# bifurcationkit/BifurcationKit.jl

Measured on NVIDIA H100. Metric: continuation steps/sec (SH2d PALC), higher is better.
Workload: dtype f64

## Files before the change

bifurcationkit.jl_b200/csrc/bk_fft_fast.cuh:

```cuda
#pragma once
#include "bk_common.cuh"
#include "bk_async.cuh"

namespace bkf {

template <int LOGN_, int LOGE_>
struct Cfg {
  static constexpr int LOGN = LOGN_, LOGE = LOGE_;
  static constexpr int N = 1 << LOGN, E = 1 << LOGE, T = N / E;
  static constexpr int F = LOGN / LOGE, RB = LOGN % LOGE;
  static constexpr int NP = F + (RB ? 1 : 0);
  static constexpr int PP = (T >= 32) ? 2 : 64 / T;
  static constexpr int THREADS = T * PP;
  static constexpr int PB = LOGE == 5 ? (LOGN >= 10 ? 5 : 4) : LOGE == 4 ? 4 : LOGE == 3 ? ((LOGN == 9 || LOGN == 10) ? 3 : 0) : 0;
  __host__ __device__ static constexpr int pad(int i) { return i + (i >> 2) + (PB ? (i >> PB) : 0); }
  static constexpr int TPSM = LOGE == 5 ? 256 : LOGE == 4 ? 512 : LOGE == 3 ? 768 : 1024;
  static constexpr int MINB = TPSM / THREADS > 0 ? TPSM / THREADS : 1;
  static constexpr int MINB_P = MINB > 1 ? MINB - 1 : 1;
  static constexpr int NB = LOGE == 2 ? (LOGN <= 6 ? 0 : LOGN <= 8 ? 4 : LOGN <= 10 ? 6 : 8)
                          : LOGE == 3 ? (LOGN <= 6 ? 0 : LOGN <= 9 ? 3 : 6)
                          : LOGE == 4 ? (LOGN <= 8 ? 0 : 4)
                                      : (LOGN <= 10 ? 0 : 5);
  __host__ __device__ static constexpr int padn(int k) { return k + (k >> 2) + (NB ? (k >> NB) : 0); }
  static constexpr int SLOTS_POS = pad(N - 1) + 1, SLOTS_NAT = padn(N - 1) + 1;
  static constexpr int SLOTS = SLOTS_POS > SLOTS_NAT ? SLOTS_POS : SLOTS_NAT;
  static constexpr size_t SMEM_DATA = sizeof(double2) * (size_t)SLOTS * PP;
  __host__ __device__ static constexpr int logr(int p) { return p < F ? LOGE : RB; }
  __host__ __device__ static constexpr int logNp(int p) { return LOGN - LOGE * p; }
  __host__ __device__ static constexpr int logMp(int p) { return logNp(p) - logr(p); }
  __host__ __device__ static constexpr int tw_off(int p) {
    int o = 0;
    for (int q = 0; q < p; ++q) o += ((1 << logr(q)) - 1) << logMp(q);
    return o;
  }
  static constexpr int TW_TOTAL = tw_off(NP);
  static constexpr size_t SMEM = SMEM_DATA + sizeof(double2) * ((size_t)TW_TOTAL + N);
  static constexpr size_t SMEM_FUSED = SMEM + sizeof(double2) * (size_t)N;
  static_assert(LOGN >= LOGE + 1 && LOGN <= 11, "line length out of range");
  static_assert(THREADS <= 1024, "CTA too large");
};

template <class C>
__host__ __device__ inline int k_of_pos(int p) {
  int k = 0, sh = 0;
  for (int q = 0; q < C::NP; ++q) {
    const int d = (p >> C::logMp(q)) & ((1 << C::logr(q)) - 1);
    k |= d << sh;
    sh += C::logr(q);
  }
  return k;
}
template <class C>
__host__ __device__ inline int pos_of_k(int k) {
  int p = 0, sh = 0;
  for (int q = 0; q < C::NP; ++q) {
    const int d = (k >> sh) & ((1 << C::logr(q)) - 1);
    p |= d << C::logMp(q);
    sh += C::logr(q);
  }
  return p;
}
__host__ __device__ constexpr int brev_c(int j, int bits) {
  int r = 0;
  for (int b = 0; b < bits; ++b) r |= ((j >> b) & 1) << (bits - 1 - b);
  return r;
}

#ifdef __CUDACC__
__device__ __forceinline__ double2 cadd(double2 a, double2 b) { return make_double2(a.x + b.x, a.y + b.y); }
__device__ __forceinline__ double2 csub(double2 a, double2 b) { return make_double2(a.x - b.x, a.y - b.y); }
__device__ __forceinline__ double2 cmul(double2 a, double2 b) {
  return make_double2(fma(a.x, b.x, -(a.y * b.y)), fma(a.x, b.y, a.y * b.x));
}
__device__ __forceinline__ double2 cmulc(double2 a, double2 b) {
  return make_double2(fma(a.x, b.x, a.y * b.y), fma(a.y, b.x, -(a.x * b.y)));
}

#define BKF_C1 0.98078528040323043
#define BKF_S1 0.19509032201612825
#define BKF_C2 0.92387953251128674
#define BKF_S2 0.38268343236508978
#define BKF_C3 0.83146961230254524
#define BKF_S3 0.55557023301960218
#define BKF_C4 0.70710678118654752
template <bool INV>
__device__ __forceinline__ double2 mul_w32(double2 t, int j) {
  double c, s;
  switch (j) {
    case 0: return t;
    case 8: return INV ? make_double2(-t.y, t.x) : make_double2(t.y, -t.x);
    case 4: {
      const double a = BKF_C4 * t.x, b = BKF_C4 * t.y;
      return INV ? make_double2(a - b, a + b) : make_double2(a + b, b - a);
    }
    case 12: {
      const double a = BKF_C4 * t.x, b = BKF_C4 * t.y;
      return INV ? make_double2(-a - b, a - b) : make_double2(b - a, -a - b);
    }
    case 1: c = BKF_C1; s = BKF_S1; break;
    case 2: c = BKF_C2; s = BKF_S2; break;
    case 3: c = BKF_C3; s = BKF_S3; break;
    case 5: c = BKF_S3; s = BKF_C3; break;
    case 6: c = BKF_S2; s = BKF_C2; break;
    case 7: c = BKF_S1; s = BKF_C1; break;
    case 9: c = -BKF_S1; s = BKF_C1; break;
    case 10: c = -BKF_S2; s = BKF_C2; break;
    case 11: c = -BKF_S3; s = BKF_C3; break;
    case 13: c = -BKF_C3; s = BKF_S3; break;
    case 14: c = -BKF_C2; s = BKF_S2; break;
    default: c = -BKF_C1; s = BKF_S1; break;
  }
  return INV ? make_double2(fma(t.x, c, -(t.y * s)), fma(t.y, c, t.x * s)) : make_double2(fma(t.x, c, t.y * s), fma(t.y, c, -(t.x * s)));
}

template <int R, int S0, int ESZ>
__device__ __forceinline__ void bfly_fwd(double2 (&a)[ESZ]) {
  if constexpr (R >= 2) {
    constexpr int H = R / 2;
#pragma unroll
    for (int i = 0; i < H; ++i) {
      const double2 u = a[S0 + i], v = a[S0 + i + H];
      a[S0 + i] = cadd(u, v);
      a[S0 + i + H] = mul_w32<false>(csub(u, v), i * (32 / R));
    }
    bfly_fwd<H, S0, ESZ>(a);
    bfly_fwd<H, S0 + H, ESZ>(a);
  }
}
template <int R, int S0, int ESZ>
__device__ __forceinline__ void bfly_inv(double2 (&a)[ESZ]) {
  if constexpr (R >= 2) {
    constexpr int H = R / 2;
    bfly_inv<H, S0, ESZ>(a);
    bfly_inv<H, S0 + H, ESZ>(a);
#pragma unroll
    for (int i = 0; i < H; ++i) {
      const double2 u = a[S0 + i], t = mul_w32<true>(a[S0 + i + H], i * (32 / R));
      a[S0 + i] = cadd(u, t);
      a[S0 + i + H] = csub(u, t);
    }
  }
}

struct Tables {
  const double2* tw;
  const double2* om;
  const double2* lam2;
};
template <class C, bool FUSED>
__device__ __forceinline__ Tables stage_tables(const Tables& g, double2* sm, unsigned long long* bar) {
  Tables t;
  double2* stw = sm + (size_t)C::SLOTS * C::PP;
  double2* som = stw + C::TW_TOTAL;
  double2* slam = som + C::N;
  if (threadIdx.x == 0) {
    mbar_init(bar, 1);
    fence_mbar_init();
    constexpr unsigned twb = 16u * C::TW_TOTAL, nb = 16u * C::N;
    mbar_arrive_expect_tx(bar, twb + nb + (FUSED ? nb : 0u));
    if (twb) bulk_g2s(stw, g.tw, twb, bar);
    bulk_g2s(som, g.om, nb, bar);
    if (FUSED) bulk_g2s(slam, g.lam2, nb, bar);
  }
  t.tw = stw;
  t.om = som;
  t.lam2 = slam;
  return t;
}

struct Geom {
  long long es;
  long long os;
  int nb;
  int nouter;
};

struct Symbol {
  const double* lam_b;
  const double* lam_o;
  double shift;
  double scale;
  const double* tail_src;
  double* tail_dst;
  int tail_n;
  int neg;
};

template <class C>
__device__ __forceinline__ int slot(int pos, int pr) { return C::pad(pos) * C::PP + pr; }

template <class C, int P>
__device__ __forceinline__ void pass_geom(int tau, int u, int& base, int& b) {
  constexpr int LM = C::logMp(P), LN = C::logNp(P);
  const int beta = tau + C::T * u;
  const int blk = beta >> LM;
  b = beta & ((1 << LM) - 1);
  base = (blk << LN) + b;
}

template <int R, int U, int NB, int ESZ>
__device__ __forceinline__ void bfly_all_fwd(double2 (&a)[ESZ]) {
  if constexpr (U < NB) {
    bfly_fwd<R, U * R, ESZ>(a);
    bfly_all_fwd<R, U + 1, NB, ESZ>(a);
  }
}
template <int R, int U, int NB, int ESZ>
__device__ __forceinline__ void bfly_all_inv(double2 (&a)[ESZ]) {
  if constexpr (U < NB) {
    bfly_inv<R, U * R, ESZ>(a);
    bfly_all_inv<R, U + 1, NB, ESZ>(a);
  }
}

template <class C, int P>
__device__ __forceinline__ void fwd_passes(double2 (&a)[C::E], double2* sm, const Tables& tb, int tau, int pr) {
  constexpr int LR = C::logr(P), R = 1 << LR, NB = C::E / R, LM = C::logMp(P);
  if constexpr (P > 0) {
#pragma unroll
    for (int u = 0; u < NB; ++u) {
      int base, b;
      pass_geom<C, P>(tau, u, base, b);
#pragma unroll
      for (int i = 0; i < R; ++i) a[u * R + i] = sm[slot<C>(base + (i << LM), pr)];
    }
  }
  bfly_all_fwd<R, 0, NB, C::E>(a);
  if constexpr (P < C::NP - 1) {
    const double2* tw = tb.tw + C::tw_off(P);
#pragma unroll
    for (int u = 0; u < NB; ++u) {
      int base, b;
      pass_geom<C, P>(tau, u, base, b);
#pragma unroll
      for (int j = 0; j < R; ++j) {
        const int q = brev_c(j, LR);
        double2 v = a[u * R + j];
        if (q > 0) v = cmul(v, tw[((q - 1) << LM) + b]);
        sm[slot<C>(base + (q << LM), pr)] = v;
      }
    }
    __syncthreads();
    fwd_passes<C, P + 1>(a, sm, tb, tau, pr);
  }
}

template <class C, int P>
__device__ __forceinline__ void inv_passes(double2 (&a)[C::E], double2* sm, const Tables& tb, int tau, int pr) {
  constexpr int LR = C::logr(P), R = 1 << LR, NB = C::E / R, LM = C::logMp(P);
  if constexpr (P < C::NP - 1) {
    const double2* tw = tb.tw + C::tw_off(P);
#pragma unroll
    for (int u = 0; u < NB; ++u) {
      int base, b;
      pass_geom<C, P>(tau, u, base, b);
#pragma unroll
      for (int j = 0; j < R; ++j) {
        const int q = brev_c(j, LR);
        double2 v = sm[slot<C>(base + (q << LM), pr)];
        if (q > 0) v = cmulc(v, tw[((q - 1) << LM) + b]);
        a[u * R + j] = v;
      }
    }
  }
  bfly_all_inv<R, 0, NB, C::E>(a);
  if constexpr (P > 0) {
#pragma unroll
    for (int u = 0; u < NB; ++u) {
      int base, b;
      pass_geom<C, P>(tau, u, base, b);
#pragma unroll
      for (int i = 0; i < R; ++i) sm[slot<C>(base + (i << LM), pr)] = a[u * R + i];
    }
    __syncthreads();
    inv_passes<C, P - 1>(a, sm, tb, tau, pr);
  }
}

template <class C>
__device__ __forceinline__ int reg_pos(int tau, int reg) {
  constexpr int LR = C::logr(C::NP - 1), R = 1 << LR;
  const int u = reg >> LR, j = reg & (R - 1);
  return ((tau + C::T * u) << LR) + brev_c(j, LR);
}
template <class C>
__device__ __forceinline__ void park(const double2 (&a)[C::E], double2* sm, int tau, int pr) {
#pragma unroll
  for (int reg = 0; reg < C::E; ++reg) sm[slot<C>(reg_pos<C>(tau, reg), pr)] = a[reg];
}
template <class C>
__device__ __forceinline__ double2 partner(const double2* sm, int pos, int pr, int& k) {
  k = k_of_pos<C>(pos);
  const int nk = (C::N - k) & (C::N - 1);
  return sm[slot<C>(pos_of_k<C>(nk), pr)];
}
template <class C>
__device__ __forceinline__ int row_of(int i, int tau) {
  const int m = i * C::T + tau;
  return (i < C::E / 2) ? 2 * m : 2 * C::N - 1 - 2 * m;
}

template <class C>
__device__ __forceinline__ void strided_load(double2 (&a)[C::E], const double* __restrict__ base, long long es, int tau, bool v0,
                                             bool v1) {
  if (v1) {
#pragma unroll
    for (int i = 0; i < C::E; ++i) a[i] = __ldg(reinterpret_cast<const double2*>(base + (long long)row_of<C>(i, tau) * es));
  } else {
#pragma unroll
    for (int i = 0; i < C::E; ++i) a[i] = make_double2(v0 ? __ldg(base + (long long)row_of<C>(i, tau) * es) : 0.0, 0.0);
  }
}
template <class C>
__device__ __forceinline__ void strided_store(const double2 (&a)[C::E], double* __restrict__ base, long long es, int tau, bool v0,
                                              bool v1) {
  if (v1) {
#pragma unroll
    for (int i = 0; i < C::E; ++i) *reinterpret_cast<double2*>(base + (long long)row_of<C>(i, tau) * es) = a[i];
  } else if (v0) {
#pragma unroll
    for (int i = 0; i < C::E; ++i) base[(long long)row_of<C>(i, tau) * es] = a[i].x;
  }
}

#define BKF_BOUNDS(C, PERIODIC) __launch_bounds__(C::THREADS, (PERIODIC) ? C::MINB_P : C::MINB)

__device__ __forceinline__ double rcp_nr(double x) {
  double r;
  asm("rcp.approx.ftz.f64 %0, %1;" : "=d"(r) : "d"(x));
  double e = fma(-x, r, 1.0);
  r = fma(r, e, r);
  e = fma(-x, r, 1.0);
  return fma(r, e, r);
}
__device__ __forceinline__ double per_symbol(const Symbol& sy, double lam) {
  const double t = 1.0 + lam, l1 = t * t;
  return sy.neg ? -sy.scale * l1 : sy.scale * rcp_nr(l1 + sy.shift);
}

template <class C, int MODE>
static __global__ void BKF_BOUNDS(C, MODE == 3) k_strided(const double* __restrict__ in, double* __restrict__ out, Geom g, Tables tbg, Symbol sy) {
  extern __shared__ __align__(128) double2 sm_fast[];
  __shared__ __align__(8) unsigned long long tbar;
  double2* sm = sm_fast;
  const Tables tb = stage_tables<C, MODE == 2 || MODE == 3>(tbg, sm, &tbar);
  const int tid = threadIdx.x, pr = tid % C::PP, tau = tid / C::PP;
  __syncthreads();
  bk_pdl_sync();
  const int col = (blockIdx.x * C::PP + pr) * 2, o = blockIdx.y;
  const bool v0 = col < g.nb, v1 = col + 1 < g.nb;
  const long long off = (long long)o * g.os + col;
  if ((MODE == 2 || MODE == 3) && sy.tail_n > 0 && blockIdx.x == 0 && blockIdx.y == 0 && tid < sy.tail_n)
    sy.tail_dst[tid] = sy.tail_src[tid];
  double2 a[C::E];
  if (MODE == 3) {
#pragma unroll
    for (int i = 0; i < C::E; ++i) {
      const double* p = in + off + (long long)(i * C::T + tau) * g.es;
      a[i] = v1 ? __ldg(reinterpret_cast<const double2*>(p)) : make_double2(v0 ? __ldg(p) : 0.0, 0.0);
    }
    mbar_wait(&tbar, 0);
    fwd_passes<C, 0>(a, sm, tb, tau, pr);
    const bool nyq = blockIdx.x == 0 && pr == 0;
    if (blockIdx.x == 0) {
      park<C>(a, sm, tau, pr);
      __syncthreads();
      if (nyq) {
        const double l0 = __ldg(sy.lam_b), ln = __ldg(sy.lam_b + (g.nb >> 1));
#pragma unroll
        for (int reg = 0; reg < C::E; ++reg) {
          int k;
          const double2 z = a[reg], zp = partner<C>(sm, reg_pos<C>(tau, reg), pr, k);
          const double ly = tb.lam2[reg * C::T + tau].x;
          const double s0 = per_symbol(sy, l0 + ly), sn = per_symbol(sy, ln + ly);
          const double hp = 0.5 * (s0 + sn), hm = 0.5 * (s0 - sn);
          a[reg] = make_double2(fma(hp, z.x, hm * zp.x), fma(hp, z.y, -(hm * zp.y)));
        }
      }
      __syncthreads();
    }
    if (!nyq) {
      const double lq = v0 ? __ldg(sy.lam_b + (col >> 1)) : 0.0;
#pragma unroll
      for (int reg = 0; reg < C::E; ++reg) {
        const double s = per_symbol(sy, lq + tb.lam2[reg * C::T + tau].x);
        a[reg] = make_double2(s * a[reg].x, s * a[reg].y);
      }
    }
    inv_passes<C, C::NP - 1>(a, sm, tb, tau, pr);
#pragma unroll
    for (int i = 0; i < C::E; ++i) {
      double* p = out + off + (long long)(i * C::T + tau) * g.es;
      if (v1) *reinterpret_cast<double2*>(p) = a[i];
      else if (v0) *p = a[i].x;
    }
    return;
  }
  if (MODE != 1) {
    strided_load<C>(a, in + off, g.es, tau, v0, v1);
    mbar_wait(&tbar, 0);
    fwd_passes<C, 0>(a, sm, tb, tau, pr);
    park<C>(a, sm, tau, pr);
    __syncthreads();
  }
  if (MODE == 0) {
#pragma unroll
    for (int reg = 0; reg < C::E; ++reg) {
      int k;
      const double2 z = a[reg], zp = partner<C>(sm, reg_pos<C>(tau, reg), pr, k);
      const double2 w = tb.om[reg * C::T + tau];
      const double sx = z.x + zp.x, sy_ = z.y - zp.y;
      const double dx = z.x - zp.x, dy = z.y + zp.y;
      const double c1 = fma(w.x, sx, -(w.y * sy_)), c2 = fma(w.x, dy, w.y * dx);
      double* p = out + off + (long long)k * g.es;
      if (v1) *reinterpret_cast<double2*>(p) = make_double2(c1, c2);
      else if (v0) *p = c1;
    }
    return;
  }
  if (MODE == 1) {
#pragma unroll
    for (int reg = 0; reg < C::E; ++reg) {
      const int k = k_of_pos<C>(reg_pos<C>(tau, reg));
      const double* p = in + off + (long long)k * g.es;
      a[reg] = v1 ? __ldg(reinterpret_cast<const double2*>(p)) : make_double2(v0 ? __ldg(p) : 0.0, 0.0);
    }
    mbar_wait(&tbar, 0);
    park<C>(a, sm, tau, pr);
    __syncthreads();
#pragma unroll
    for (int reg = 0; reg < C::E; ++reg) {
      int k;
      double2 dn = partner<C>(sm, reg_pos<C>(tau, reg), pr, k);
      if (k == 0) dn = make_double2(0.0, 0.0);
      const double2 w = tb.om[reg * C::T + tau];
      a[reg] = cmulc(make_double2(a[reg].x + dn.y, a[reg].y - dn.x), w);
    }
    __syncthreads();
  }
  if (MODE == 2) {
    const double lo = sy.lam_o ? __ldg(sy.lam_o + o) : 0.0;
    const double cA = 1.0 + lo + (v0 ? __ldg(sy.lam_b + col) : 0.0), cB = 1.0 + lo + (v1 ? __ldg(sy.lam_b + col + 1) : 0.0);
#pragma unroll
    for (int reg = 0; reg < C::E; ++reg) {
      int k;
      const double2 z = a[reg], zp = partner<C>(sm, reg_pos<C>(tau, reg), pr, k);
      const double2 w = tb.om[reg * C::T + tau];
      const double2 l2 = tb.lam2[reg * C::T + tau];
      const double2 A1 = cmul(make_double2(z.x + zp.x, z.y - zp.y), w);
      const double2 A2 = cmul(make_double2(z.y + zp.y, zp.x - z.x), w);
      double t = cA + l2.x;
      const double s1k = fma(t, t, sy.shift);
      t = cA + l2.y;
      const double s1n = fma(t, t, sy.shift);
      t = cB + l2.x;
      const double s2k = fma(t, t, sy.shift);
      t = cB + l2.y;
      const double s2n = fma(t, t, sy.shift);
      const double r1 = sy.scale * __drcp_rn(s1k * s1n), r2 = sy.scale * __drcp_rn(s2k * s2n);
      const double h1x = A1.x * (r1 * s1n), h1y = A1.y * (r1 * s1k);
      const double h2x = A2.x * (r2 * s2n), h2y = A2.y * (r2 * s2k);
      a[reg] = cmulc(make_double2(h1x - h2y, h1y + h2x), w);
    }
    __syncthreads();
  }
  inv_passes<C, C::NP - 1>(a, sm, tb, tau, pr);
  strided_store<C>(a, out + off, g.es, tau, v0, v1);
}

template <class C>
__device__ __forceinline__ int nslot(int k, int pr) { return C::padn(k) * C::PP + pr; }

__device__ __forceinline__ double pw_c(const PerPw& pw, double u) { return fma(u, fma(-3.0, u, 2.0 * pw.nu), pw.l); }
__device__ __forceinline__ double pw_d(const PerPw& pw, double u) { return fma(pw.a1, pw.spc + pw_c(pw, u), pw.a0); }
__device__ __forceinline__ double pw_out(const PerPw& pw, double y, const double* v, const double* u, int m, double s) {
  switch (pw.epi) {
    case PW_RESID: {
      const double x = __ldg(v + m);
      return fma(x, fma(x, pw.nu - x, pw.l), y);
    }
    case PW_JVP: return fma(fma(pw.a1, pw_c(pw, __ldg(u + m)), pw.a0), s * __ldg(v + m), y);
    case PW_FLEFT: return fma(-pw.a1 * s, __ldg(v + m), y);
    case PW_FRIGHT: return fma(pw_d(pw, __ldg(u + m)), y, -pw.a1 * s * __ldg(v + m));
    default: return y;
  }
}

template <class C, int MODE>
static __global__ void BKF_BOUNDS(C, MODE == 2) k_contig(const double* __restrict__ in, double* __restrict__ out, Geom g, Tables tbg, PerPw pw) {
  extern __shared__ __align__(128) double2 sm_fast[];
  __shared__ __align__(8) unsigned long long tbar;
  double2* sm = sm_fast;
  const Tables tb = stage_tables<C, false>(tbg, sm, &tbar);
  const int tid = threadIdx.x, pr = tid % C::PP, tau = tid / C::PP;
  __syncthreads();
  bk_pdl_sync();
  const long long lineA = ((long long)blockIdx.x * C::PP + pr) * 2, lineB = lineA + 1;
  const bool vA = lineA < g.nb, vB = lineB < g.nb;
  const double* inA = in + lineA * g.os;
  const double* inB = in + lineB * g.os;
  double* outA = out + lineA * g.os;
  double* outB = out + lineB * g.os;
  double2 a[C::E];
  if (MODE == 2) {
    const double s = pw.sp ? __ldg(pw.sp) : 1.0;
#pragma unroll
    for (int i = 0; i < C::E; ++i) {
      const int m = i * C::T + tau;
      double xa = vA ? __ldg(inA + m) : 0.0, xb = vB ? __ldg(inB + m) : 0.0;
      if (pw.pro == PW_D) {
        xa *= vA ? pw_d(pw, __ldg(pw.u + lineA * g.os + m)) : 0.0;
        xb *= vB ? pw_d(pw, __ldg(pw.u + lineB * g.os + m)) : 0.0;
      }
      a[i] = make_double2(s * xa, s * xb);
    }
    mbar_wait(&tbar, 0);
    fwd_passes<C, 0>(a, sm, tb, tau, pr);
    park<C>(a, sm, tau, pr);
    __syncthreads();
    double2 b[C::E];
#pragma unroll
    for (int reg = 0; reg < C::E; ++reg) {
      int k;
      const double2 z = a[reg], zp = partner<C>(sm, reg_pos<C>(tau, reg), pr, k);
      a[reg] = make_double2(0.5 * (z.x + zp.x), 0.5 * (z.y + zp.y));
      b[reg] = make_double2(0.5 * (z.y - zp.y), 0.5 * (zp.x - z.x));
    }
    __syncthreads();
#pragma unroll
    for (int reg = 0; reg < C::E; ++reg) {
      const int k = k_of_pos<C>(reg_pos<C>(tau, reg));
      if (k == 0) sm[nslot<C>(0, pr)] = a[reg];
      else if (k == C::N / 2) sm[nslot<C>(1, pr)] = a[reg];
      else if (k < C::N / 2) {
        sm[nslot<C>(2 * k, pr)] = a[reg];
        sm[nslot<C>(2 * k + 1, pr)] = b[reg];
      }
    }
    __syncthreads();
#pragma unroll
    for (int i = 0; i < C::E; ++i) {
      const int p = i * C::T + tau;
      const double2 d = sm[nslot<C>(p, pr)];
      if (vA) outA[p] = d.x;
      if (vB) outB[p] = d.y;
    }
    return;
  }
  if (MODE == 3) {
#pragma unroll
    for (int i = 0; i < C::E; ++i) {
      const int p = i * C::T + tau;
      sm[nslot<C>(p, pr)] = make_double2(vA ? __ldg(inA + p) : 0.0, vB ? __ldg(inB + p) : 0.0);
    }
    mbar_wait(&tbar, 0);
    __syncthreads();
#pragma unroll
    for (int reg = 0; reg < C::E; ++reg) {
      const int k = k_of_pos<C>(reg_pos<C>(tau, reg)), kk = k <= C::N / 2 ? k : C::N - k;
      double2 xa, xb;
      if (kk == 0 || kk == C::N / 2) {
        const double2 d = sm[nslot<C>(kk ? 1 : 0, pr)];
        xa = make_double2(d.x, 0.0);
        xb = make_double2(d.y, 0.0);
      } else {
        const double2 re = sm[nslot<C>(2 * kk, pr)], im = sm[nslot<C>(2 * kk + 1, pr)];
        xa = make_double2(re.x, k == kk ? im.x : -im.x);
        xb = make_double2(re.y, k == kk ? im.y : -im.y);
      }
      a[reg] = make_double2(xa.x - xb.y, xa.y + xb.x);
    }
    __syncthreads();
    inv_passes<C, C::NP - 1>(a, sm, tb, tau, pr);
    const double s = pw.sp ? __ldg(pw.sp) : 1.0;
    const double* vrA = pw.v + lineA * g.os;
    const double* vrB = pw.v + lineB * g.os;
    const double* urA = pw.u ? pw.u + lineA * g.os : nullptr;
    const double* urB = pw.u ? pw.u + lineB * g.os : nullptr;
#pragma unroll
    for (int i = 0; i < C::E; ++i) {
      const int m = i * C::T + tau;
      if (vA) outA[m] = pw_out(pw, a[i].x, vrA, urA, m, s);
      if (vB) outB[m] = pw_out(pw, a[i].y, vrB, urB, m, s);
    }
    return;
  }
  if (MODE == 0) {
#pragma unroll
    for (int i = 0; i < C::E; ++i) {
      const int e = row_of<C>(i, tau);
      a[i] = make_double2(vA ? __ldg(inA + e) : 0.0, vB ? __ldg(inB + e) : 0.0);
    }
    mbar_wait(&tbar, 0);
    fwd_passes<C, 0>(a, sm, tb, tau, pr);
    park<C>(a, sm, tau, pr);
    __syncthreads();
#pragma unroll
    for (int reg = 0; reg < C::E; ++reg) {
      int k;
      const double2 z = a[reg], zp = partner<C>(sm, reg_pos<C>(tau, reg), pr, k);
      const double2 w = tb.om[reg * C::T + tau];
      const double sx = z.x + zp.x, sy_ = z.y - zp.y, dx = z.x - zp.x, dy = z.y + zp.y;
      a[reg] = make_double2(fma(w.x, sx, -(w.y * sy_)), fma(w.x, dy, w.y * dx));
    }
    __syncthreads();
#pragma unroll
    for (int reg = 0; reg < C::E; ++reg) sm[nslot<C>(k_of_pos<C>(reg_pos<C>(tau, reg)), pr)] = a[reg];
    __syncthreads();
#pragma unroll
    for (int i = 0; i < C::E; ++i) {
      const int k = i * C::T + tau;
      const double2 d = sm[nslot<C>(k, pr)];
      if (vA) outA[k] = d.x;
      if (vB) outB[k] = d.y;
    }
  } else {
#pragma unroll
    for (int i = 0; i < C::E; ++i) {
      const int k = i * C::T + tau;
      sm[nslot<C>(k, pr)] = make_double2(vA ? __ldg(inA + k) : 0.0, vB ? __ldg(inB + k) : 0.0);
    }
    mbar_wait(&tbar, 0);
    __syncthreads();
#pragma unroll
    for (int reg = 0; reg < C::E; ++reg) {
      const int k = k_of_pos<C>(reg_pos<C>(tau, reg)), nk = (C::N - k) & (C::N - 1);
      const double2 w = tb.om[reg * C::T + tau];
      const double2 d = sm[nslot<C>(k, pr)];
      double2 dn = sm[nslot<C>(nk, pr)];
      if (k == 0) dn = make_double2(0.0, 0.0);
      a[reg] = cmulc(make_double2(d.x + dn.y, d.y - dn.x), w);
    }
    __syncthreads();
    inv_passes<C, C::NP - 1>(a, sm, tb, tau, pr);
#pragma unroll
    for (int i = 0; i < C::E; ++i) {
      const int e = row_of<C>(i, tau);
      if (vA) outA[e] = a[i].x;
      if (vB) outB[e] = a[i].y;
    }
  }
}
#endif

template <class C>
static inline void build_tables(std::vector<double>& tw, std::vector<double>& om, std::vector<double>& lam2, const double* lam) {
  const long double PI = 3.14159265358979323846264338327950288L;
  tw.assign(2 * (size_t)C::TW_TOTAL, 0.0);
  for (int p = 0; p < C::NP - 1; ++p) {
    const int r = 1 << C::logr(p), M = 1 << C::logMp(p), Np = 1 << C::logNp(p);
    for (int q = 1; q < r; ++q)
      for (int b = 0; b < M; ++b) {
        const long double ang = -2.0L * PI * (long double)((long long)b * q % Np) / Np;
        const size_t i = (size_t)C::tw_off(p) + (size_t)(q - 1) * M + b;
        tw[2 * i] = (double)cosl(ang);
        tw[2 * i + 1] = (double)sinl(ang);
      }
  }
  om.assign(2 * (size_t)C::N, 0.0);
  lam2.assign(2 * (size_t)C::N, 0.0);
  const int LR = C::logr(C::NP - 1), R = 1 << LR;
  for (int reg = 0; reg < C::E; ++reg)
    for (int tau = 0; tau < C::T; ++tau) {
      const int u = reg >> LR, j = reg & (R - 1);
      const int pos = ((tau + C::T * u) << LR) + brev_c(j, LR);
      const int k = k_of_pos<C>(pos), nk = (C::N - k) & (C::N - 1);
      const size_t i = (size_t)reg * C::T + tau;
      om[2 * i] = (double)cosl(-PI * k / (2.0L * C::N));
      om[2 * i + 1] = (double)sinl(-PI * k / (2.0L * C::N));
      if (lam) {
        lam2[2 * i] = lam[k];
        lam2[2 * i + 1] = lam[nk];
      }
    }
}
}
```

bifurcationkit.jl_b200/csrc/bk_precond.cu:

```cuda
#include <cmath>
#include <cstdlib>
#include <utility>
#include <vector>
#include "bk_common.cuh"

#include "bk_fft_fast.cuh"
#include "bk_fft_gen.cuh"

static __global__ void __launch_bounds__(256) k_sh_symbol_div(double* __restrict__ a, int nx, int ny, int nz,
                                                              const double* __restrict__ lx, const double* __restrict__ ly,
                                                              const double* __restrict__ lz, double shift, double scale) {
  const long long total = (long long)nx * ny * nz;
  for (long long q = (long long)blockIdx.x * blockDim.x + threadIdx.x; q < total; q += (long long)gridDim.x * blockDim.x) {
    int i = (int)(q % nx), j = (int)((q / nx) % ny), k = (int)(q / ((long long)nx * ny));
    double t = 1.0 + lx[i] + ly[j] + (lz ? lz[k] : 0.0);
    a[q] = a[q] * scale / (t * t + shift);
  }
}
static __global__ void __launch_bounds__(256) k_helmholtz_symbol_div(double* __restrict__ a, int nx, int ny, long long nblocks,
                                                                     const double* __restrict__ lx,
                                                                     const double* __restrict__ ly, double a0, double a1) {
  const long long n = (long long)nx * ny, total = n * nblocks;
  for (long long q = (long long)blockIdx.x * blockDim.x + threadIdx.x; q < total; q += (long long)gridDim.x * blockDim.x) {
    long long g = q % n;
// ... 37 lines not shown
    const double dp = 1.0 / (sp.x * sp.x + sp.y * sp.y), dm = 1.0 / (sm.x * sm.x + sm.y * sm.y);
    yp[k] = make_double2((ap.x * sp.x + ap.y * sp.y) * dp * invK, (ap.y * sp.x - ap.x * sp.y) * dp * invK);
    ym[k] = make_double2((am.x * sm.x + am.y * sm.y) * dm * invK, (am.y * sm.x - am.x * sm.y) * dm * invK);
  }
  for (int i = 0; i < K; ++i) {
    double2 ap = make_double2(0, 0), am = make_double2(0, 0);
    int idx = 0;
    for (int k = 0; k < K; ++k) {
      const double2 t = tw[idx];
      ap.x += yp[k].x * t.x + yp[k].y * t.y;
      ap.y += yp[k].y * t.x - yp[k].x * t.y;
      am.x += ym[k].x * t.x + ym[k].y * t.y;
      am.y += ym[k].y * t.x - ym[k].x * t.y;
      idx += i;
      if (idx >= K) idx -= K;
    }
    B[(long long)(2 * i) * n + g] = 0.5 * (ap.x + am.x);
    B[(long long)(2 * i + 1) * n + g] = 0.5 * (ap.y - am.y);
  }
}
static __global__ void __launch_bounds__(128) k_potrap_time_tr(double* __restrict__ B, long long n, int nx, int K,
                                                               const double* __restrict__ lamx, const double* __restrict__ lamy,
                                                               double h, double r, double nu, const double2* __restrict__ tw) {
  const long long g = (long long)blockIdx.x * blockDim.x + threadIdx.x;
  if (g >= n) return;
  const double lam = lamx[g % nx] + lamy[g / nx];
  double2 wp[BK_PO_KMAX], wm[BK_PO_KMAX];
  for (int i = 0; i < K; ++i) {
    double a = B[(long long)(2 * i) * n + g], b = B[(long long)(2 * i + 1) * n + g];
    if (i == 0) {
      a += B[(long long)(2 * K) * n + g];
      b += B[(long long)(2 * K + 1) * n + g];
    }
    wp[i] = make_double2(a, b);
    wm[i] = make_double2(a, -b);
  }
  double2 yp[BK_PO_KMAX], ym[BK_PO_KMAX];
  const double invK = 1.0 / K;
  for (int k = 0; k < K; ++k) {
    double2 ap = make_double2(0, 0), am = make_double2(0, 0);
    int idx = 0;
    for (int i = 0; i < K; ++i) {
      const double2 t = tw[idx];
      ap.x += wp[i].x * t.x - wp[i].y * t.y;
      ap.y += wp[i].x * t.y + wp[i].y * t.x;
      am.x += wm[i].x * t.x - wm[i].y * t.y;
      am.y += wm[i].x * t.y + wm[i].y * t.x;
      idx += k;
      if (idx >= K) idx -= K;
    }
    const double2 gk = tw[k];
    const double2 omg = make_double2(1.0 - gk.x, -gk.y), opg = make_double2(1.0 + gk.x, gk.y);
    const double cr = lam + r;
    double2 sp = make_double2(omg.x - 0.5 * h * (opg.x * cr - opg.y * nu), omg.y - 0.5 * h * (opg.x * nu + opg.y * cr));
    double2 sm = make_double2(omg.x - 0.5 * h * (opg.x * cr + opg.y * nu), omg.y - 0.5 * h * (-opg.x * nu + opg.y * cr));
    sp.y = -sp.y;
    sm.y = -sm.y;
    const double dp = 1.0 / (sp.x * sp.x + sp.y * sp.y), dm = 1.0 / (sm.x * sm.x + sm.y * sm.y);
    yp[k] = make_double2((ap.x * sp.x + ap.y * sp.y) * dp * invK, (ap.y * sp.x - ap.x * sp.y) * dp * invK);
    ym[k] = make_double2((am.x * sm.x + am.y * sm.y) * dm * invK, (am.y * sm.x - am.x * sm.y) * dm * invK);
  }
  for (int i = 0; i < K; ++i) {
    double2 ap = make_double2(0, 0), am = make_double2(0, 0);
    int idx = 0;
    for (int k = 0; k < K; ++k) {
      const double2 t = tw[idx];
      ap.x += yp[k].x * t.x + yp[k].y * t.y;
      ap.y += yp[k].y * t.x - yp[k].x * t.y;
      am.x += ym[k].x * t.x + ym[k].y * t.y;
      am.y += ym[k].y * t.x - ym[k].x * t.y;
      idx += i;
      if (idx >= K) idx -= K;
    }
    B[(long long)(2 * i) * n + g] = 0.5 * (ap.x + am.x);
    B[(long long)(2 * i + 1) * n + g] = 0.5 * (ap.y - am.y);
  }
}
static __global__ void __launch_bounds__(256) k_potrap_close(const double* __restrict__ in, double* __restrict__ out,
                                                             long long Ns, int M) {
  const long long i = (long long)blockIdx.x * blockDim.x + threadIdx.x;
  if (i < Ns) out[(long long)(M - 1) * Ns + i] = in[(long long)(M - 1) * Ns + i] + out[i];
  if (i == 0) out[(long long)M * Ns] = in[(long long)M * Ns];
}

static __global__ void k_thomas(const double* __restrict__ tri, const double* __restrict__ in, double* __restrict__ out, int n) {
  if (blockIdx.x != 0 || threadIdx.x != 0) return;
  const double* cp = tri;
  const double* di = tri + n;
  const double* lo = tri + 2 * n;
  double prev = in[0] * di[0];
  out[0] = prev;
  for (int i = 1; i < n; ++i) {
    prev = (in[i] - lo[i] * prev) * di[i];
    out[i] = prev;
  }
  for (int i = n - 2; i >= 0; --i) out[i] -= cp[i] * out[i + 1];
}

static int upload(bk_ctx* c, void** dst, const void* src, size_t bytes) {
  if (*dst) cudaFree(*dst);
  *dst = nullptr;
  BK_CUDA(c, cudaMalloc(dst, bytes));
  BK_CUDA(c, cudaMemcpy(*dst, src, bytes, cudaMemcpyHostToDevice));
  return BK_OK;
}

static int fast_loge(long long n) {
  static int e = -1;
  if (e < 0) {
    const char* a = getenv("BK_FFT_LOGE");
    e = a ? atoi(a) : 0;
    if (e < 2 || e > 5) e = 0;
  }
  if (e) return e;
  return n >= 1024 ? 3 : 2;
}
static int fast_logn(long long n) {
  static int off = -1;
  if (off < 0) off = getenv("BK_FFT_NO_FAST") ? 1 : 0;
  if (off) return 0;
  for (int l = fast_loge(n) + 1; l <= 11; ++l)
    if (l >= 6 && n == (1LL << l)) return l;
  return 0;
}
#define BKF_DISPATCH_N(LE, LOGN, ...)                                                   \
  switch (LOGN) {                                                                      \
    case 6: { using FC = bkf::Cfg<6, LE>; __VA_ARGS__; } break;                        \
    case 7: { using FC = bkf::Cfg<7, LE>; __VA_ARGS__; } break;                        \
    case 8: { using FC = bkf::Cfg<8, LE>; __VA_ARGS__; } break;                        \
    case 9: { using FC = bkf::Cfg<9, LE>; __VA_ARGS__; } break;                        \
    case 10: { using FC = bkf::Cfg<10, LE>; __VA_ARGS__; } break;                      \
    default: { using FC = bkf::Cfg<11, LE>; __VA_ARGS__; } break;                      \
  }
#define BKF_DISPATCH(LOGN, ...)                                                        \
  switch (fast_loge(1LL << (LOGN))) {                                                               \
    case 2: BKF_DISPATCH_N(2, LOGN, __VA_ARGS__) break;                                \
    case 3: BKF_DISPATCH_N(3, LOGN, __VA_ARGS__) break;                                \
    case 4: BKF_DISPATCH_N(4, LOGN, __VA_ARGS__) break;                                \
    default: BKF_DISPATCH_N(5, LOGN, __VA_ARGS__) break;                               \
  }

template <class FC>
static int fast_setup(bk_ctx* c, int d, const double* lam_host) {
  std::vector<double> tw, om, lam2;
  bkf::build_tables<FC>(tw, om, lam2, lam_host);
  Precond& pc = c->pc;
  if (tw.empty()) tw.assign(2, 0.0);
  BK_TRY(upload(c, (void**)&pc.ftw[d], tw.data(), 8 * tw.size()));
  BK_TRY(upload(c, (void**)&pc.fom[d], om.data(), 8 * om.size()));
  BK_TRY(upload(c, (void**)&pc.flam2[d], lam2.data(), 8 * lam2.size()));
  return BK_OK;
}

template <class FC>
static int fast_launch(bk_ctx* c, int d, bool strided, int mode, const double* in, double* out, const bkf::Geom& g,
                       const bkf::Symbol* sy, const PerPw* pw = nullptr) {
  Precond& pc = c->pc;
  bkf::Tables tb{pc.ftw[d], pc.fom[d], pc.flam2[d]};
  bkf::Symbol s0{};
  if (sy) s0 = *sy;
  PerPw p0{};
  if (pw) p0 = *pw;
  if (strided) {
    static decltype(&bkf::k_strided<FC, 0>) const kern[4] = {bkf::k_strided<FC, 0>, bkf::k_strided<FC, 1>, bkf::k_strided<FC, 2>,
                                                             bkf::k_strided<FC, 3>};
    const dim3 grid((g.nb + 2 * FC::PP - 1) / (2 * FC::PP), g.nouter);
    return bk_launch(c, kern[mode], grid, dim3(FC::THREADS), mode >= 2 ? FC::SMEM_FUSED : FC::SMEM, in, out, g, tb, s0);
  }
  static decltype(&bkf::k_contig<FC, 0>) const kern[4] = {bkf::k_contig<FC, 0>, bkf::k_contig<FC, 1>, bkf::k_contig<FC, 2>,
                                                          bkf::k_contig<FC, 3>};
  const dim3 grid((unsigned)((g.nb + 2 * FC::PP - 1) / (2 * FC::PP)));
  return bk_launch(c, kern[mode], grid, dim3(FC::THREADS), FC::SMEM, in, out, g, tb, p0);
}

static void factorize(int L, bkg::Plan& pl) {
  pl.npass = 0;
  while (L % 4 == 0 && pl.npass < BKG_MAXPASS) {
    pl.radix[pl.npass++] = 4;
    L /= 4;
  }
  for (int p = 2; L > 1 && pl.npass < BKG_MAXPASS; ++p)
    while (L % p == 0 && pl.npass < BKG_MAXPASS) {
      pl.radix[pl.npass++] = p;
      L /= p;
    }
}
#define BKG_THREADS 512
#define BKG_SMEM_BUDGET (100 * 1024)
#define BKG_SMEM_MAX (200 * 1024)
static int gen_ppg(int L) {
  long long per = 32LL * L;
  int p = (int)(BKG_SMEM_BUDGET / per);
  if (p < 1) p = 1;
  if (p > 8) p = 8;
  return p;
}

static int gen_setup(bk_ctx* c, int d, int n, int type) {
  Precond& pc = c->pc;
  bkg::Plan& pl = pc.gplan[d];
  pl.n = n;
  pl.L = type == 0 ? 2 * n : 2 * n + 2;
  BK_CHECK(c, 32LL * pl.L <= BKG_SMEM_MAX, "line too long for the general transform kernel (n <= 3199)");
  factorize(pl.L, pl);
  const long double PI = 3.14159265358979323846264338327950288L;
  std::vector<double> wl(2 * (size_t)pl.L), ph(2 * (size_t)n);
  for (int t = 0; t < pl.L; ++t) {
    wl[2 * t] = (double)cosl(-2.0L * PI * t / pl.L);
    wl[2 * t + 1] = (double)sinl(-2.0L * PI * t / pl.L);
  }
  for (int k = 0; k < n; ++k) {
    ph[2 * k] = (double)cosl(-PI * k / (2.0L * n));
    ph[2 * k + 1] = (double)sinl(-PI * k / (2.0L * n));
  }
  BK_TRY(upload(c, (void**)&pc.gwl[d], wl.data(), 8 * wl.size()));
  BK_TRY(upload(c, (void**)&pc.gph[d], ph.data(), 8 * ph.size()));
  pl.wl = pc.gwl[d];
  pl.ph = pc.gph[d];
  pl.dst_scale = 0.5 * sqrt(2.0 / (n + 1.0));
  return BK_OK;
}

static int gen_launch(bk_ctx* c, int d, bool strided, int mode, const double* in, double* out, const bkf::Geom& g) {
  const bkg::Plan& pl = c->pc.gplan[d];
  const int ppg = gen_ppg(pl.L);
  const size_t sm = 32 * (size_t)pl.L * ppg;
  const long long npairs = ((long long)g.nb + 1) / 2;
  dim3 grid((unsigned)((npairs + ppg - 1) / ppg), strided ? g.nouter : 1);
  static decltype(&bkg::k_gen<false, 0>) const kern[2][3] = {{bkg::k_gen<false, 0>, bkg::k_gen<false, 1>, bkg::k_gen<false, 2>},
                                                              {bkg::k_gen<true, 0>, bkg::k_gen<true, 1>, bkg::k_gen<true, 2>}};
  return bk_launch(c, kern[strided][mode], grid, dim3(BKG_THREADS), sm, in, out, g, pl, ppg);
}

static int setup_dim(bk_ctx* c, int d, long long n, double inv_h2, int type, bool even_nx) {
  Precond& pc = c->pc;
  std::vector<double> lam(n);
  const long double PI = 3.14159265358979323846264338327950288L;
  for (long long k = 0; k < n; ++k)
    lam[k] = (type == 0) ? (double)((2.0L * cosl(PI * k / n) - 2.0L)) * inv_h2
                         : (double)(-(2.0L - 2.0L * cosl(PI * (k + 1) / (n + 1)))) * inv_h2;
  BK_TRY(upload(c, (void**)&pc.lam[d], lam.data(), 8 * n));
  pc.ttype[d] = type;
  pc.fast[d] = (type == 0 && even_nx) ? fast_logn(n) : 0;
  if (pc.fast[d]) {
    BKF_DISPATCH(pc.fast[d], BK_TRY(fast_setup<FC>(c, d, lam.data())));
  }
  return gen_setup(c, d, (int)n, type);
}

int bk_periodic_setup(bk_ctx* c) {
  Precond& pc = c->pc;
  const long double PI = 3.14159265358979323846264338327950288L;
  for (int d = 0; d < 2; ++d) {
    const long long n = c->dims[d];
    int logn = 0;
    while ((1LL << logn) < n) ++logn;
    std::vector<double> lam(n);
    for (long long k = 0; k < n; ++k) {
      const long double ks = (long double)(k <= n / 2 ? k : k - n), w = PI * ks / (long double)c->lengths[d];
      lam[k] = (double)(-w * w);
    }
    BK_TRY(upload(c, (void**)&pc.lam[d], lam.data(), 8 * n));
    pc.fast[d] = logn;
    BKF_DISPATCH(logn, BK_TRY(fast_setup<FC>(c, d, lam.data())));
  }
  if (!pc.work) BK_CUDA(c, cudaMalloc(&pc.work, 8 * (size_t)c->ld));
  if (!pc.work2) BK_CUDA(c, cudaMalloc(&pc.work2, 8 * (size_t)c->ld));
  return BK_OK;
}

static int periodic_pipeline(bk_ctx* c, const double* in, double* out, const PerPw& pw, bool neg, double gain, double shift,
                             const double* tail_src = nullptr, double* tail_dst = nullptr, int tail_n = 0) {
  Precond& pc = c->pc;
  const int nx = (int)c->dims[0], ny = (int)c->dims[1];
  const bkf::Geom gx{1, nx, ny, 1}, gy{nx, (long long)nx * ny, nx, 1};
  const bkf::Symbol sy{pc.lam[0], nullptr, shift, gain / ((double)nx * (double)ny), tail_src, tail_dst, tail_n, neg ? 1 : 0};
  BKF_DISPATCH(pc.fast[0], BK_TRY(fast_launch<FC>(c, 0, false, 2, in, pc.work, gx, nullptr, &pw)));
  BKF_DISPATCH(pc.fast[1], BK_TRY(fast_launch<FC>(c, 1, true, 3, pc.work, pc.work2, gy, &sy)));
  BKF_DISPATCH(pc.fast[0], BK_TRY(fast_launch<FC>(c, 0, false, 3, pc.work2, out, gx, nullptr, &pw)));
  return BK_OK;
}

int bk_periodic_residual(bk_ctx* c, const OpDesc& op, const double* u, double* out) {
  const PerPw pw{0, PW_RESID, u, nullptr, nullptr, 0.0, 0.0, op.par[0], op.par[1], 0.0};
  return periodic_pipeline(c, u, out, pw, true, 1.0, 0.0);
}
int bk_periodic_jvp(bk_ctx* c, const OpDesc& op, const double* in, const double* sp, double* out) {
  const PerPw pw{0, PW_JVP, in, op.u, sp, op.a0, op.a1, op.par[0], op.par[1], 0.0};
  return periodic_pipeline(c, in, out, pw, true, op.a1, 0.0);
}
int bk_periodic_fused(bk_ctx* c, const OpDesc& op, const double* in, const double* sp, double* out, bool left) {
  BK_CHECK(c, c->pc.kind == BK_PC_SH_FFT && !op.bordered && !op.cplx, "internal: one-transform operator needs BK_PC_SH_FFT, unbordered, real");
  const PerPw pw{left ? PW_D : 0, left ? PW_FLEFT : PW_FRIGHT, in, op.u, sp, op.a0, op.a1, op.par[0], op.par[1], c->pc.a0};
  return periodic_pipeline(c, in, out, pw, false, 1.0, c->pc.a0);
}

extern "C" int32_t bk_precond_setup(bk_ctx* c, int32_t kind, double a0, double a1) {
  BK_ENTER(c);
  BK_CUDA(c, cudaStreamSynchronize(c->stream));
  Precond& pc = c->pc;
  if (kind == BK_PC_NONE) {
    pc.kind = BK_PC_NONE;
    return BK_OK;
  }
  if (!pc.work) BK_CUDA(c, cudaMalloc(&pc.work, 8 * (size_t)c->ld));
  if (!pc.work2) BK_CUDA(c, cudaMalloc(&pc.work2, 8 * (size_t)c->ld));
  const bool even_nx = (c->dims[0] % 2) == 0;
  if (kind == BK_PC_SH_DCT) {
    BK_CHECK(c, c->kind == BK_SH2D || c->kind == BK_SH3D, "BK_PC_SH_DCT needs a Swift-Hohenberg context");
    for (int d = 0; d < bk_kind_traits(c->kind)->ndims; ++d) BK_TRY(setup_dim(c, d, c->dims[d], bk_inv_h2(c, d), 0, even_nx));
  } else if (kind == BK_PC_SH_FFT) {
    BK_CHECK(c, c->kind == BK_SH2D_PERIODIC, "BK_PC_SH_FFT needs a BK_SH2D_PERIODIC context");
    BK_CHECK(c, a0 > 0, "BK_PC_SH_FFT: a0 must be > 0 (the symbol of L1 vanishes at |k| = 1)");
  } else if (kind == BK_PC_CGL_DST) {
    BK_CHECK(c, c->kind == BK_CGL2D || c->kind == BK_POTRAP_CGL2D, "BK_PC_CGL_DST needs a cGL context");
    for (int d = 0; d < 2; ++d) BK_TRY(setup_dim(c, d, c->dims[d], bk_inv_h2(c, d), 1, even_nx));
  } else if (kind == BK_PC_POTRAP_CIRC) {
    BK_CHECK(c, c->kind == BK_POTRAP_CGL2D, "BK_PC_POTRAP_CIRC needs a Trapeze (potrap) context");
    const int K = (int)c->dims[2] - 1;
    BK_CHECK(c, K >= 1 && K <= BK_PO_KMAX, "BK_PC_POTRAP_CIRC supports 2 <= M <= 65 time slices");
    BK_CHECK(c, a0 > 0, "BK_PC_POTRAP_CIRC: a0 must be the period T > 0");
    for (int d = 0; d < 2; ++d) BK_TRY(setup_dim(c, d, c->dims[d], bk_inv_h2(c, d), 1, even_nx));
    std::vector<double2> tw(K);
    const long double PI = 3.14159265358979323846264338327950288L;
    for (int j = 0; j < K; ++j) tw[j] = make_double2((double)cosl(-2.0L * PI * j / K), (double)sinl(-2.0L * PI * j / K));
// ... 188 lines not shown
```

Measured before the change: 4.375.

## Make fast FFT transform kernels persistent with occupancy-sized grids

Wraps the strided and contiguous FFT kernel bodies in device functions and launches grid-stride persistent kernels sized to the occupancy limit times the SM count. Each block then stages its twiddle tables into shared memory once and reuses them across several work units, instead of every block paying that staging cost. Launch-bound minimum-blocks hints change for several modes (a new MINB_S for non-periodic strided kernels, swapped hints for contig), which alters register limits. The trade-off is an extra __syncthreads per unit and possible load imbalance across blocks.

```diff
diff --git a/bifurcationkit.jl_b200/csrc/bk_fft_fast.cuh b/bifurcationkit.jl_b200/csrc/bk_fft_fast.cuh
--- a/bifurcationkit.jl_b200/csrc/bk_fft_fast.cuh
+++ b/bifurcationkit.jl_b200/csrc/bk_fft_fast.cuh
@@ -17,6 +17,7 @@
   static constexpr int TPSM = LOGE == 5 ? 256 : LOGE == 4 ? 512 : LOGE == 3 ? 768 : 1024;
   static constexpr int MINB = TPSM / THREADS > 0 ? TPSM / THREADS : 1;
   static constexpr int MINB_P = MINB > 1 ? MINB - 1 : 1;
+  static constexpr int MINB_S = MINB * 3 / 4 > 0 ? MINB * 3 / 4 : 1;
   static constexpr int NB = LOGE == 2 ? (LOGN <= 6 ? 0 : LOGN <= 8 ? 4 : LOGN <= 10 ? 6 : 8)
                           : LOGE == 3 ? (LOGN <= 6 ? 0 : LOGN <= 9 ? 3 : 6)
                           : LOGE == 4 ? (LOGN <= 8 ? 0 : 4)
@@ -323,7 +324,7 @@
   }
 }
 
-#define BKF_BOUNDS(C, PERIODIC) __launch_bounds__(C::THREADS, (PERIODIC) ? C::MINB_P : C::MINB)
+#define BKF_BOUNDS(C, MINB_) __launch_bounds__(C::THREADS, MINB_)
 
 __device__ __forceinline__ double rcp_nr(double x) {
   double r;
@@ -339,18 +340,13 @@
 }
 
 template <class C, int MODE>
-static __global__ void BKF_BOUNDS(C, MODE == 3) k_strided(const double* __restrict__ in, double* __restrict__ out, Geom g, Tables tbg, Symbol sy) {
-  extern __shared__ __align__(128) double2 sm_fast[];
-  __shared__ __align__(8) unsigned long long tbar;
-  double2* sm = sm_fast;
-  const Tables tb = stage_tables<C, MODE == 2 || MODE == 3>(tbg, sm, &tbar);
+__device__ __forceinline__ void strided_unit(const double* __restrict__ in, double* __restrict__ out, const Geom& g, const Tables& tb,
+                                             const Symbol& sy, double2* sm, unsigned long long* tbar, int x, int o) {
   const int tid = threadIdx.x, pr = tid % C::PP, tau = tid / C::PP;
-  __syncthreads();
-  bk_pdl_sync();
-  const int col = (blockIdx.x * C::PP + pr) * 2, o = blockIdx.y;
+  const int col = (x * C::PP + pr) * 2;
   const bool v0 = col < g.nb, v1 = col + 1 < g.nb;
   const long long off = (long long)o * g.os + col;
-  if ((MODE == 2 || MODE == 3) && sy.tail_n > 0 && blockIdx.x == 0 && blockIdx.y == 0 && tid < sy.tail_n)
+  if ((MODE == 2 || MODE == 3) && sy.tail_n > 0 && x == 0 && o == 0 && tid < sy.tail_n)
     sy.tail_dst[tid] = sy.tail_src[tid];
   double2 a[C::E];
   if (MODE == 3) {
@@ -359,10 +355,10 @@
       const double* p = in + off + (long long)(i * C::T + tau) * g.es;
       a[i] = v1 ? __ldg(reinterpret_cast<const double2*>(p)) : make_double2(v0 ? __ldg(p) : 0.0, 0.0);
     }
-    mbar_wait(&tbar, 0);
+    mbar_wait(tbar, 0);
     fwd_passes<C, 0>(a, sm, tb, tau, pr);
-    const bool nyq = blockIdx.x == 0 && pr == 0;
-    if (blockIdx.x == 0) {
+    const bool nyq = x == 0 && pr == 0;
+    if (x == 0) {
       park<C>(a, sm, tau, pr);
       __syncthreads();
       if (nyq) {
@@ -398,7 +394,7 @@
   }
   if (MODE != 1) {
     strided_load<C>(a, in + off, g.es, tau, v0, v1);
-    mbar_wait(&tbar, 0);
+    mbar_wait(tbar, 0);
     fwd_passes<C, 0>(a, sm, tb, tau, pr);
     park<C>(a, sm, tau, pr);
     __syncthreads();
@@ -425,7 +421,7 @@
       const double* p = in + off + (long long)k * g.es;
       a[reg] = v1 ? __ldg(reinterpret_cast<const double2*>(p)) : make_double2(v0 ? __ldg(p) : 0.0, 0.0);
     }
-    mbar_wait(&tbar, 0);
+    mbar_wait(tbar, 0);
     park<C>(a, sm, tau, pr);
     __syncthreads();
 #pragma unroll
@@ -468,6 +464,21 @@
   strided_store<C>(a, out + off, g.es, tau, v0, v1);
 }
 
+template <class C, int MODE>
+static __global__ void BKF_BOUNDS(C, MODE == 3 ? C::MINB_P : C::MINB_S) k_strided(const double* __restrict__ in, double* __restrict__ out, Geom g, Tables tbg, Symbol sy) {
+  extern __shared__ __align__(128) double2 sm_fast[];
+  __shared__ __align__(8) unsigned long long tbar;
+  double2* sm = sm_fast;
+  const Tables tb = stage_tables<C, MODE == 2 || MODE == 3>(tbg, sm, &tbar);
+  __syncthreads();
+  bk_pdl_sync();
+  const int nbx = (g.nb + 2 * C::PP - 1) / (2 * C::PP), units = nbx * g.nouter;
+  for (int u = blockIdx.x; u < units; u += gridDim.x) {
+    strided_unit<C, MODE>(in, out, g, tb, sy, sm, &tbar, u % nbx, u / nbx);
+    __syncthreads();
+  }
+}
+
 template <class C>
 __device__ __forceinline__ int nslot(int k, int pr) { return C::padn(k) * C::PP + pr; }
 
@@ -487,15 +498,10 @@
 }
 
 template <class C, int MODE>
-static __global__ void BKF_BOUNDS(C, MODE == 2) k_contig(const double* __restrict__ in, double* __restrict__ out, Geom g, Tables tbg, PerPw pw) {
-  extern __shared__ __align__(128) double2 sm_fast[];
-  __shared__ __align__(8) unsigned long long tbar;
-  double2* sm = sm_fast;
-  const Tables tb = stage_tables<C, false>(tbg, sm, &tbar);
+__device__ __forceinline__ void contig_unit(const double* __restrict__ in, double* __restrict__ out, const Geom& g, const Tables& tb,
+                                            const PerPw& pw, double2* sm, unsigned long long* tbar, int x) {
   const int tid = threadIdx.x, pr = tid % C::PP, tau = tid / C::PP;
-  __syncthreads();
-  bk_pdl_sync();
-  const long long lineA = ((long long)blockIdx.x * C::PP + pr) * 2, lineB = lineA + 1;
+  const long long lineA = ((long long)x * C::PP + pr) * 2, lineB = lineA + 1;
   const bool vA = lineA < g.nb, vB = lineB < g.nb;
   const double* inA = in + lineA * g.os;
   const double* inB = in + lineB * g.os;
@@ -514,7 +520,7 @@
       }
       a[i] = make_double2(s * xa, s * xb);
     }
-    mbar_wait(&tbar, 0);
+    mbar_wait(tbar, 0);
     fwd_passes<C, 0>(a, sm, tb, tau, pr);
     park<C>(a, sm, tau, pr);
     __syncthreads();
@@ -553,7 +559,7 @@
       const int p = i * C::T + tau;
       sm[nslot<C>(p, pr)] = make_double2(vA ? __ldg(inA + p) : 0.0, vB ? __ldg(inB + p) : 0.0);
     }
-    mbar_wait(&tbar, 0);
+    mbar_wait(tbar, 0);
     __syncthreads();
 #pragma unroll
     for (int reg = 0; reg < C::E; ++reg) {
@@ -591,7 +597,7 @@
       const int e = row_of<C>(i, tau);
       a[i] = make_double2(vA ? __ldg(inA + e) : 0.0, vB ? __ldg(inB + e) : 0.0);
     }
-    mbar_wait(&tbar, 0);
+    mbar_wait(tbar, 0);
     fwd_passes<C, 0>(a, sm, tb, tau, pr);
     park<C>(a, sm, tau, pr);
     __syncthreads();
@@ -620,7 +626,7 @@
       const int k = i * C::T + tau;
       sm[nslot<C>(k, pr)] = make_double2(vA ? __ldg(inA + k) : 0.0, vB ? __ldg(inB + k) : 0.0);
     }
-    mbar_wait(&tbar, 0);
+    mbar_wait(tbar, 0);
     __syncthreads();
 #pragma unroll
     for (int reg = 0; reg < C::E; ++reg) {
@@ -639,6 +645,21 @@
       if (vA) outA[e] = a[i].x;
       if (vB) outB[e] = a[i].y;
     }
+  }
+}
+
+template <class C, int MODE>
+static __global__ void BKF_BOUNDS(C, MODE == 3 ? C::MINB : C::MINB_P) k_contig(const double* __restrict__ in, double* __restrict__ out, Geom g, Tables tbg, PerPw pw) {
+  extern __shared__ __align__(128) double2 sm_fast[];
+  __shared__ __align__(8) unsigned long long tbar;
+  double2* sm = sm_fast;
+  const Tables tb = stage_tables<C, false>(tbg, sm, &tbar);
+  __syncthreads();
+  bk_pdl_sync();
+  const int units = (g.nb + 2 * C::PP - 1) / (2 * C::PP);
+  for (int u = blockIdx.x; u < units; u += gridDim.x) {
+    contig_unit<C, MODE>(in, out, g, tb, pw, sm, &tbar, u);
+    __syncthreads();
   }
 }
 #endif
diff --git a/bifurcationkit.jl_b200/csrc/bk_precond.cu b/bifurcationkit.jl_b200/csrc/bk_precond.cu
--- a/bifurcationkit.jl_b200/csrc/bk_precond.cu
+++ b/bifurcationkit.jl_b200/csrc/bk_precond.cu
@@ -213,6 +213,20 @@
   return BK_OK;
 }
 
+template <class K>
+static int persistent_grid(bk_ctx* c, K kern, int threads, size_t smem, long long units, int* per_sm, unsigned* grid) {
+  if (!*per_sm) {
+    bk_ensure_smem(c, kern, smem);
+    int r = 0;
+    BK_CUDA(c, cudaOccupancyMaxActiveBlocksPerMultiprocessor(&r, kern, threads, smem));
+    BK_CHECK(c, r >= 1, "internal: transform kernel does not fit on an SM");
+    *per_sm = r;
+  }
+  const long long slots = (long long)*per_sm * c->nsm;
+  *grid = (unsigned)(units < slots ? units : slots);
+  return BK_OK;
+}
+
 template <class FC>
 static int fast_launch(bk_ctx* c, int d, bool strided, int mode, const double* in, double* out, const bkf::Geom& g,
                        const bkf::Symbol* sy, const PerPw* pw = nullptr) {
@@ -222,16 +236,21 @@
   if (sy) s0 = *sy;
   PerPw p0{};
   if (pw) p0 = *pw;
+  const long long units = (g.nb + 2 * FC::PP - 1) / (2 * FC::PP) * (strided ? g.nouter : 1);
+  static int per_sm[2][4] = {};
   if (strided) {
     static decltype(&bkf::k_strided<FC, 0>) const kern[4] = {bkf::k_strided<FC, 0>, bkf::k_strided<FC, 1>, bkf::k_strided<FC, 2>,
                                                              bkf::k_strided<FC, 3>};
-    const dim3 grid((g.nb + 2 * FC::PP - 1) / (2 * FC::PP), g.nouter);
-    return bk_launch(c, kern[mode], grid, dim3(FC::THREADS), mode >= 2 ? FC::SMEM_FUSED : FC::SMEM, in, out, g, tb, s0);
+    const size_t smem = mode >= 2 ? FC::SMEM_FUSED : FC::SMEM;
+    unsigned grid;
+    BK_TRY(persistent_grid(c, kern[mode], FC::THREADS, smem, units, &per_sm[1][mode], &grid));
+    return bk_launch(c, kern[mode], dim3(grid), dim3(FC::THREADS), smem, in, out, g, tb, s0);
   }
   static decltype(&bkf::k_contig<FC, 0>) const kern[4] = {bkf::k_contig<FC, 0>, bkf::k_contig<FC, 1>, bkf::k_contig<FC, 2>,
                                                           bkf::k_contig<FC, 3>};
-  const dim3 grid((unsigned)((g.nb + 2 * FC::PP - 1) / (2 * FC::PP)));
-  return bk_launch(c, kern[mode], grid, dim3(FC::THREADS), FC::SMEM, in, out, g, tb, p0);
+  unsigned grid;
+  BK_TRY(persistent_grid(c, kern[mode], FC::THREADS, FC::SMEM, units, &per_sm[0][mode], &grid));
+  return bk_launch(c, kern[mode], dim3(grid), dim3(FC::THREADS), FC::SMEM, in, out, g, tb, p0);
 }
 
 static void factorize(int L, bkg::Plan& pl) {
```

After: 4.385, median of 6. About the same (+0.2%).
